# MarcoLor01/SparseMatrixVectorMultiplication

Measured on AMD Instinct MI355X. Metric: SpMV GFLOP/s (2*nnz flops / step time); achieved HBM GB/s and % of 8 TB/s alongside, higher is better.
Workload: dtype f64

## Files before the change

include/spmv_hip.h:

```cpp
#ifndef SPMV_AMD_SPMV_HIP_H
#define SPMV_AMD_SPMV_HIP_H

#include <stddef.h>

#include "csr_matrix.h"
#include "hll_matrix.h"

#ifdef __cplusplus
extern "C" {
#endif

typedef struct spmv_csr_dev spmv_csr_dev;
typedef struct spmv_hll_dev spmv_hll_dev;

enum {
    SPMV_CSR_AUTO = 0,
    SPMV_CSR_THREAD_ROW = 1,
    SPMV_CSR_WAVE_ROW = 2,
    SPMV_CSR_SUBWAVE = 3,
    SPMV_CSR_STREAM = 4
};

enum {
    SPMV_HLL_AUTO = 0,
// ... 31 lines not shown
    int tile_long_items;
    long long tile_long_entries;
    long long tile_staged_cols;
    long long tile_remainder_entries;
    int tile_mid_rows;
    int tile_mid_items;
    long long tile_mid_entries;
    int place_tries;
    float place_first_us;
    float place_best_us;
    unsigned long long val_address;
    long long tile_expanded_entries;
    long long pattern_slots;
    float pattern_with_us;
    float pattern_without_us;
} spmv_dev_info;

int spmv_hip_device_count(void);
int spmv_hip_init(int device);
int spmv_hip_shutdown(void);
int spmv_hip_sync(void);
void *spmv_hip_stream(void);
const char *spmv_hip_last_error(void);
int spmv_hip_device_name(char *buf, size_t len, int *compute_units, long long *hbm_bytes);
int spmv_hip_flush_cache(size_t bytes);
int spmv_hip_device_state(char *buf, size_t len);
int spmv_hip_stream_probe(size_t bytes, int warmup, int iters, float *ms_mean, float *ms_min);
int spmv_hip_stream_probe_at(const void *dptr, size_t bytes, int warmup, int iters, float *ms_mean, float *ms_min);
int spmv_hip_gather_probe(int value_bytes, size_t table_bytes, int waves_per_cu, double *values_per_s);
int spmv_hip_set_tuning(const char *key, int value);
// ... 10 lines not shown
                            const float *values, int row0, int row1, spmv_csr_dev **out);
int spmv_hip_csr_plan_check(int M, int N, const int *row_ptr, const int *col_idx, int value_bytes, int *stats);
int spmv_hip_csr_tile_plan_check(int M, int N, const int *row_ptr, const int *col_idx, int value_bytes,
                                 int rows_per_block, int lmax, int density, int chunk, int balance, long long *stats);
int spmv_hip_csr_tile_auto_plan(int M, int N, const int *row_ptr, const int *col_idx, int value_bytes, long long *stats);
int spmv_hip_csr_tile_digest(const spmv_csr_dev *m, unsigned long long *digest);
int spmv_hip_hll_tile_digest(const spmv_hll_dev *m, unsigned long long *digest);
int spmv_hip_csr_from_coo(int M, int N, long long nz, const int *I, const int *J, const double *val,
                          spmv_csr_dev **out);
int spmv_hip_csr_download(const spmv_csr_dev *m, int *row_ptr, int *col, void *val);
int spmv_hip_csr_upload_matrix(const CSRMatrix *csr, spmv_csr_dev **out);
void spmv_hip_csr_free(spmv_csr_dev *m);
int spmv_hip_csr_info(const spmv_csr_dev *m, spmv_dev_info *out);
int spmv_hip_csr_addresses(const spmv_csr_dev *m, unsigned long long *out);
int spmv_hip_csr_stamp_blocks(spmv_csr_dev *m, int warm, unsigned long long *stamps);
int spmv_hip_csr_relocate(spmv_csr_dev *m, int which, unsigned long long align, unsigned long long offset);
int spmv_hip_csr_relocate_vmm(spmv_csr_dev *m, int which, unsigned long long align, unsigned long long offset);

int spmv_hip_csr_set_x(spmv_csr_dev *m, const void *x_host);
int spmv_hip_csr_run(spmv_csr_dev *m, int variant);
int spmv_hip_csr_get_y(spmv_csr_dev *m, void *y_host);
void *spmv_hip_csr_x_ptr(spmv_csr_dev *m);
void *spmv_hip_csr_y_ptr(spmv_csr_dev *m);

int spmv_hip_csr_run_on(spmv_csr_dev *m, int variant, const void *d_x, void *d_y, void *stream);

int spmv_hip_csr_spmm_on(spmv_csr_dev *m, int k, const void *d_X, void *d_Y, void *stream);
int spmv_hip_csr_spmm(spmv_csr_dev *m, int k, const void *X_host, void *Y_host);
int spmv_hip_csr_spmm_time(spmv_csr_dev *m, int k, int warmup, int iters, float *ms_each);

// ... 67 lines not shown
```

sparsematrixvectormultiplication_amd/_native.py:

```python
from __future__ import annotations

import ctypes as C
import os

_HERE = os.path.dirname(os.path.abspath(__file__))
LIB_PATH = os.path.join(_HERE, "libspmv_amd.so")

c_int_p = C.POINTER(C.c_int)
c_double_p = C.POINTER(C.c_double)
c_float_p = C.POINTER(C.c_float)


class PreMatrix(C.Structure):
    _fields_ = [("M", C.c_int), ("N", C.c_int), ("nz", C.c_int), ("I", c_int_p), ("J", c_int_p),
                ("val", c_double_p), ("type", C.c_char * 4)]


class CSRMatrix(C.Structure):
    _fields_ = [("M", C.c_int), ("N", C.c_int), ("nz", C.c_int), ("row_ptr", c_int_p),
                ("col_idx", c_int_p), ("values", c_double_p), ("type", C.c_char * 4)]


class ELLPACKBlock(C.Structure):
    _fields_ = [("M", C.c_int), ("N", C.c_int), ("MAXNZ", C.c_int), ("JA", c_int_p),
# ... 11 lines not shown

class DevInfo(C.Structure):
    _fields_ = [("M_local", C.c_int), ("M_total", C.c_int), ("N", C.c_int), ("row0", C.c_int),
                ("nz", C.c_longlong), ("value_bytes", C.c_int), ("auto_variant", C.c_int),
                ("lanes_per_row", C.c_int), ("stream_blocks", C.c_int), ("long_rows", C.c_int),
                ("slots", C.c_longlong), ("hacks", C.c_int), ("algo_bytes", C.c_longlong),
                ("device_bytes", C.c_longlong), ("local_blocks", C.c_int), ("local_stage_lines", C.c_int),
                ("local_lines", C.c_longlong), ("stream_bytes", C.c_longlong), ("stream_kernel", C.c_int),
                ("tile_blocks", C.c_int), ("tile_passes", C.c_int), ("tile_split_rows", C.c_int),
                ("tile_entries", C.c_longlong), ("tile_staged_entries", C.c_longlong),
                ("tile_long_rows", C.c_int), ("tile_long_items", C.c_int), ("tile_long_entries", C.c_longlong),
                ("tile_staged_cols", C.c_longlong), ("tile_remainder_entries", C.c_longlong),
                ("tile_mid_rows", C.c_int), ("tile_mid_items", C.c_int), ("tile_mid_entries", C.c_longlong),
                ("place_tries", C.c_int), ("place_first_us", C.c_float), ("place_best_us", C.c_float),
                ("val_address", C.c_ulonglong), ("tile_expanded_entries", C.c_longlong),
                ("pattern_slots", C.c_longlong), ("pattern_with_us", C.c_float), ("pattern_without_us", C.c_float)]

    def as_dict(self):
        return {name: getattr(self, name) for name, _ in self._fields_}


_PROTOTYPES = {
    "mm_read_banner": (C.c_int, [C.c_void_p, C.c_void_p]),
    "mm_read_mtx_crd_size": (C.c_int, [C.c_void_p, c_int_p, c_int_p, c_int_p]),
    "mm_write_banner": (C.c_int, [C.c_void_p, C.c_char_p]),
    "mm_write_mtx_crd_size": (C.c_int, [C.c_void_p, C.c_int, C.c_int, C.c_int]),
    "mm_is_valid": (C.c_int, [C.c_char_p]),
    "mm_typecode_to_str": (C.c_void_p, [C.c_char_p]),
    "init_pre_matrix": (None, [C.POINTER(PreMatrix)]),
    "free_pre_matrix": (None, [C.POINTER(PreMatrix)]),
    "read_matrix_market": (C.c_int, [C.c_char_p, C.POINTER(PreMatrix)]),
# ... 59 lines not shown
    "spmv_hip_init": (C.c_int, [C.c_int]),
    "spmv_hip_shutdown": (C.c_int, []),
    "spmv_hip_sync": (C.c_int, []),
    "spmv_hip_stream": (C.c_void_p, []),
    "spmv_hip_last_error": (C.c_char_p, []),
    "spmv_hip_device_name": (C.c_int, [C.c_char_p, C.c_size_t, c_int_p, C.POINTER(C.c_longlong)]),
    "spmv_hip_flush_cache": (C.c_int, [C.c_size_t]),
    "spmv_hip_device_state": (C.c_int, [C.c_char_p, C.c_size_t]),
    "spmv_hip_stream_probe": (C.c_int, [C.c_size_t, C.c_int, C.c_int, c_float_p, c_float_p]),
    "spmv_hip_stream_probe_at": (C.c_int, [C.c_void_p, C.c_size_t, C.c_int, C.c_int, c_float_p, c_float_p]),
    "spmv_hip_gather_probe": (C.c_int, [C.c_int, C.c_size_t, C.c_int, c_double_p]),
    "spmv_hip_csr_tile_digest": (C.c_int, [C.c_void_p, C.POINTER(C.c_ulonglong)]),
    "spmv_hip_hll_tile_digest": (C.c_int, [C.c_void_p, C.POINTER(C.c_ulonglong)]),
    "spmv_hip_csr_addresses": (C.c_int, [C.c_void_p, C.POINTER(C.c_ulonglong)]),
    "spmv_hip_csr_stamp_blocks": (C.c_int, [C.c_void_p, C.c_int, C.POINTER(C.c_ulonglong)]),
    "spmv_hip_csr_relocate": (C.c_int, [C.c_void_p, C.c_int, C.c_ulonglong, C.c_ulonglong]),
    "spmv_hip_csr_relocate_vmm": (C.c_int, [C.c_void_p, C.c_int, C.c_ulonglong, C.c_ulonglong]),
    "spmv_hip_set_tuning": (C.c_int, [C.c_char_p, C.c_int]),
    "spmv_hip_malloc": (C.c_int, [C.POINTER(C.c_void_p), C.c_size_t]),
    "spmv_hip_free": (C.c_int, [C.c_void_p]),
    "spmv_hip_memcpy_h2d": (C.c_int, [C.c_void_p, C.c_void_p, C.c_size_t]),
    "spmv_hip_memcpy_d2h": (C.c_int, [C.c_void_p, C.c_void_p, C.c_size_t]),
    "spmv_hip_memset": (C.c_int, [C.c_void_p, C.c_int, C.c_size_t]),
    "spmv_hip_csr_upload": (C.c_int, [C.c_int, C.c_int, c_int_p, c_int_p, c_double_p, C.c_int,
                                      C.c_int, C.POINTER(C.c_void_p)]),
    "spmv_hip_csr_upload_f32": (C.c_int, [C.c_int, C.c_int, c_int_p, c_int_p, c_float_p, C.c_int,
                                          C.c_int, C.POINTER(C.c_void_p)]),
    "spmv_hip_csr_upload_matrix": (C.c_int, [C.POINTER(CSRMatrix), C.POINTER(C.c_void_p)]),
    "spmv_hip_csr_free": (None, [C.c_void_p]),
    "spmv_hip_csr_info": (C.c_int, [C.c_void_p, C.POINTER(DevInfo)]),
# ... 92 lines not shown
```

sparsematrixvectormultiplication_amd/csrc/hip/csr_kernels.hpp:

```cpp
#pragma once
#include <hip/hip_runtime.h>

#include <type_traits>

#include "wave_ops.hpp"

namespace spmv {

constexpr int kBlock = 256;
constexpr int kStreamCapMax = 8192;
constexpr int kStreamUnit = 2 * kBlock;
constexpr int kStreamRowsCap = 1024;
constexpr int kLongPiece = 8192;
constexpr int kBaseMask = ~3;

typedef int v2i __attribute__((ext_vector_type(2)));
typedef float v2f __attribute__((ext_vector_type(2)));
typedef double v2d __attribute__((ext_vector_type(2)));
template <typename T> struct vec2;
template <> struct vec2<float> { using type = v2f; };
template <> struct vec2<double> { using type = v2d; };

template <bool NT, typename V>
__device__ __forceinline__ V stream_load(const V *p) {
// ... 452 lines not shown
#pragma unroll
    for (int k = 0; k < ROUNDS; ++k)
        *reinterpret_cast<uint4 *>(reinterpret_cast<char *>(stage) + (k * kBlock + t) * 16) = xl[k];
    __syncthreads();
#pragma unroll
    for (int u = 0; u < kUnits; ++u) {
        const unsigned c = *reinterpret_cast<const unsigned *>(pc.slots + u * kUnit + 2 * t);
        v[u].x *= stage[c & 0xffffu];
        v[u].y *= stage[c >> 16];
    }
    __syncthreads();
#pragma unroll
    for (int u = 0; u < kUnits; ++u) *reinterpret_cast<V2 *>(&stage[u * kUnit + 2 * t]) = v[u];
}

template <typename T, bool NT, int CAP, bool STAMP = false, bool PAT = false>
__global__ __launch_bounds__(kBlock) void csr_stream_local(int num_blocks, int xcd_chunk,
                                                           const int *__restrict__ ids,
                                                           const int4 *__restrict__ desc,
                                                           const int2 *__restrict__ ldesc,
                                                           const int *__restrict__ lines,
                                                           const int *__restrict__ row_ptr,
                                                           const unsigned short *__restrict__ lcol,
                                                           const T *__restrict__ val,
                                                           const T *__restrict__ x, T *__restrict__ y,
                                                           unsigned long long *__restrict__ stamps = nullptr, int probe = 0,
                                                           const int2 *__restrict__ pdesc = nullptr,
                                                           const unsigned *__restrict__ rinfo = nullptr,
                                                           const unsigned short *__restrict__ ptab = nullptr, int stage_bytes = 0) {
        using V2 = typename vec2<T>::type;
    const bool no_slots = STAMP && (probe & 1);
    unsigned long long t_start = 0;
    if constexpr (STAMP) t_start = __builtin_amdgcn_s_memrealtime();
    constexpr int kUnit = 2 * kBlock, kUnits = CAP / kUnit;
    extern __shared__ __attribute__((aligned(16))) unsigned char local_smem[];
    T *stage = reinterpret_cast<T *>(local_smem);

    const int at = xcd_chunked(blockIdx.x, xcd_chunk);
    if (at >= num_blocks) return;
    const int b = ids ? ids[at] : at;
    const int t = threadIdx.x;
    const int4 d = desc[b];
    const int2 ld = ldesc[b];
    const int r0 = d.x, nrows = d.z;
    const int base = d.y & kBaseMask;

    const int lanes = lanes_for_rows<kBlock>(nrows);
    int seg_lo = 0, seg_hi = 0;
    if (t / lanes < nrows) {
        seg_lo = row_ptr[r0 + t / lanes];
        seg_hi = row_ptr[r0 + t / lanes + 1];
    }

    const int e_first = base + 2 * t;
    const int units = (d.w - base + kUnit - 1) / kUnit;
    const int rounds = (ld.y + kLocalLineQuantum - 1) / kLocalLineQuantum;
    const int *my_lines = lines + ld.x;
    if constexpr (PAT) {
        const int2 pd = pdesc[b];
        pat_ctx pc;
        pc.slots = reinterpret_cast<unsigned short *>(local_smem + stage_bytes);
        pc.ptab8 = reinterpret_cast<const uint4 *>(ptab + pd.x);
        pc.rinfo = rinfo;
        pc.row_ptr = row_ptr;
        pc.row_seg = nullptr;
        pc.r0 = r0;
        pc.nrows = nrows;
        pc.base = base;
        pc.first = d.y;
        pc.end = d.w;
        pc.lanes = lanes;
        pc.seg_lo = seg_lo;
        pc.seg_hi = seg_hi;
        pc.ri = t / lanes < nrows ? rinfo[r0 + t / lanes] : 0u;
        if (units == kUnits) {
            switch (rounds) {
// ... 55 lines not shown
#pragma unroll
        for (int u = 0; u < kUnits; ++u) {
            if (u < units) {
                const unsigned c = stream_load<NT>(reinterpret_cast<const unsigned *>(lcol + e_first + u * kUnit));
                p[u] = stream_load<NT>(reinterpret_cast<const V2 *>(val + e_first + u * kUnit));
                p[u].x *= stage[c & 0xffffu];
                p[u].y *= stage[c >> 16];
            }
        }
        __syncthreads();
#pragma unroll
        for (int u = 0; u < kUnits; ++u)
            if (u < units) *reinterpret_cast<V2 *>(&stage[u * kUnit + 2 * t]) = p[u];
    }
    __syncthreads();
    sum_rows_from_lds<T, kBlock>(stage, row_ptr, y, r0, nrows, base, lanes, seg_lo - base, seg_hi - base);
    if constexpr (STAMP) {
        __syncthreads();
        if (threadIdx.x == 0) {
            stamps[3 * (size_t)b] = t_start;
            stamps[3 * (size_t)b + 1] = __builtin_amdgcn_s_memrealtime();
            stamps[3 * (size_t)b + 2] = ((unsigned long long)blockIdx.x << 8) | (__builtin_amdgcn_s_getreg(20 | (3 << 11)) & 0xf);
        }
    }
}

template <typename T, bool NT>
__global__ __launch_bounds__(kBlock) void csr_long_pieces(int count, const int4 *__restrict__ pieces,
                                                          const int *__restrict__ col,
                                                          const T *__restrict__ val,
                                                          const T *__restrict__ x,
// ... 63 lines not shown
```

sparsematrixvectormultiplication_amd/csrc/hip/plan_kernels.hpp:

```cpp
#pragma once
#include <hip/hip_runtime.h>

#include <climits>

#include "csr_kernels.hpp"

namespace spmv {

constexpr int kPlanCap = 2048;
constexpr int kPlanPer = kPlanCap / kBlock;

template <int SHIFT>
__device__ __forceinline__ int sort_segment_lines(int *keys, int *scan, const int *__restrict__ idx, long long begin,
                                                  int len) {
    const int t = threadIdx.x;
#pragma unroll
    for (int j = 0; j < kPlanPer; ++j) {
        const int k = t + j * kBlock;
        keys[k] = k < len ? (idx[begin + k] >> SHIFT) : INT_MAX;
    }
    for (int size = 2; size <= kPlanCap; size <<= 1) {
        for (int stride = size >> 1; stride > 0; stride >>= 1) {
            __syncthreads();
#pragma unroll
// ... 167 lines not shown
            rinfo[r0 + i] = (unsigned)cur | ((unsigned)(shift & 0xffff) << 16);
        }
        pdesc[b] = make_int2((int)pb, filled * 8);
    }
    __syncthreads();
    for (int i = t; i < nrows; i += BLOCK) {
        if (rowflag[r0 + i] & 0x10000) continue;
        long long s;
        int len;
        pat_row_slots<HLL>(row_ptr, row_seg, base, r0 + i, s, len);
        const long long o = pb + 8 * (long long)(rinfo[r0 + i] & 0xffffu);
        for (int j = 0; j < len; ++j) ptab[o + j] = slot[s + j];
    }
}

}
```

sparsematrixvectormultiplication_amd/csrc/hip/spmv_csr.hip:

```cpp
#include "spmv_internal.hpp"

#include "plan_kernels.hpp"
#include <chrono>

#include "tile_plan.hpp"
#include "tile_plan_device.hpp"

namespace {

void csr_build_blocks(int M, const int *rp, int cap, int rows_cap, std::vector<int4> &desc,
                      std::vector<int4> &pieces, std::vector<int4> &long_rows,
                      const std::vector<unsigned char> *split = nullptr) {
    desc.clear();
    pieces.clear();
    long_rows.clear();
    auto is_long = [&](int row) { return rp[row + 1] - rp[row] > cap - 3 || (split && (*split)[row]); };
    int r = 0;
    while (r < M) {
        const int n0 = rp[r];
        const int base = n0 & kBaseMask;
        if (is_long(r)) {
            const int first_slot = (int)pieces.size();
            for (int p = n0; p < rp[r + 1]; p += kLongPiece)
                pieces.push_back(int4{r, p, std::min(p + kLongPiece, rp[r + 1]), (int)pieces.size()});
// ... 624 lines not shown
            best_us = us;
        }
        worst_us = std::max(worst_us, us);
        if (best_us < worst_us * 0.915f) break;
    }
    m->val = best;
    m->place_best_us = best_us;
    if (best != first) (void)hipFree(first);
    for (void *p : others)
        if (p != best) (void)hipFree(p);
    (void)hipEventDestroy(e0);
    (void)hipEventDestroy(e1);
    return rc;
}

int csr_build_patterns(spmv_csr_dev *m) {
    if (g_local_patterns == 0 || m->local_blocks <= 0 || !m->lcol || !m->ldesc4 || !m->row_ptr || m->M_local <= 0) return 0;
    if (g_local_patterns < 0 && (m->nz * (m->value_bytes + 2LL) <= (128LL << 20) || m->nz < 12LL * m->M_local)) return 0;
    UploadTrace trace("csr_build_patterns");
    const int B = m->local_blocks;
    int *rowflag = nullptr, *pcount = nullptr;
    long long *pbase = nullptr;
    auto drop_tmp = [&] {
        (void)hipFree(rowflag);
        (void)hipFree(pcount);
        (void)hipFree(pbase);
    };
    hipError_t e = hipMalloc((void **)&rowflag, (size_t)m->M_local * sizeof(int));
    if (e == hipSuccess) e = hipMalloc((void **)&pcount, (size_t)B * sizeof(int));
    if (e == hipSuccess) e = hipMalloc((void **)&pbase, (size_t)B * sizeof(long long));
// ... 12 lines not shown
        return fail("pattern plan: marking the rows failed: %s", hipGetErrorString(e));
    }
    std::vector<long long> h_base((size_t)B);
    long long total = 0;
    int widest = 0;
    for (int b = 0; b < B; ++b) {
        h_base[(size_t)b] = total;
        total += h_count[(size_t)b];
        widest = std::max(widest, h_count[(size_t)b]);
    }
    trace.mark("rows marked");
    if ((g_local_patterns < 0 && total * 4 > m->nz) || total > 0x7ffffff0LL) {
        drop_tmp();
        return 0;
    }
    e = hipMalloc((void **)&m->ptab, ((size_t)total + 1024) * sizeof(unsigned short));
    if (e == hipSuccess) e = hipMalloc((void **)&m->rinfo, (size_t)m->M_local * sizeof(unsigned));
    if (e == hipSuccess) e = hipMalloc((void **)&m->pdesc, (size_t)B * sizeof(int2));
    if (e == hipSuccess) e = hipMemsetAsync(m->ptab, 0, ((size_t)total + 1024) * sizeof(unsigned short), g_stream);
    if (e == hipSuccess) e = hipMemsetAsync(m->rinfo, 0, (size_t)m->M_local * sizeof(unsigned), g_stream);
    if (e == hipSuccess) e = hipMemcpyAsync(pbase, h_base.data(), (size_t)B * sizeof(long long), hipMemcpyHostToDevice, g_stream);
    if (e == hipSuccess) {
        hipLaunchKernelGGL((pat_fill<256>), dim3(B), dim3(256), 0, g_stream, B, m->ldesc4, m->row_ptr, m->lcol, rowflag, pbase, m->rinfo,
                           m->ptab, m->pdesc);
        e = hipGetLastError();
    }
    if (e == hipSuccess) e = hipStreamSynchronize(g_stream);
    drop_tmp();
    if (e != hipSuccess) {
        (void)hipFree(m->ptab);
        (void)hipFree(m->rinfo);
        (void)hipFree(m->pdesc);
        m->ptab = nullptr;
        m->rinfo = nullptr;
        m->pdesc = nullptr;
        return fail("pattern plan: building the tables failed: %s", hipGetErrorString(e));
    }
    m->pat_slots = total;
    m->pat_max = widest;
    m->device_bytes += ((size_t)total + 1024) * 2 + (size_t)m->M_local * 4 + (size_t)B * 8;
    trace.mark("tables");
    return 0;
}

int csr_tune_patterns(spmv_csr_dev *m) {
    if (g_local_patterns >= 0 || !m->ptab || !m->x || !m->y) return 0;
    hipEvent_t e0 = nullptr, e1 = nullptr;
    if (hipEventCreate(&e0) != hipSuccess || hipEventCreate(&e1) != hipSuccess) {
        if (e0) (void)hipEventDestroy(e0);
        return 0;
    }
    auto measure = [&](int patterns, float &us) {
        const int keep = g_local_patterns;
        g_local_patterns = patterns;
        int rc = 0;
        for (int i = 0; i < 2 && !rc; ++i) rc = csr_launch_any(m, SPMV_CSR_AUTO, m->x, m->y, g_stream);
// ... 8 lines not shown
        return (e == hipSuccess && !rc) ? 0 : -1;
    };
    float with_us = 0, without_us = 0;
    bool ok = true;
    for (int round = 0; round < 2 && ok; ++round) {
        float a = 0, b = 0;
        ok = measure(1, a) == 0 && measure(0, b) == 0;
        with_us = round ? std::min(with_us, a) : a;
        without_us = round ? std::min(without_us, b) : b;
    }
    (void)hipEventDestroy(e0);
    (void)hipEventDestroy(e1);
    m->pat_with_us = with_us;
    m->pat_without_us = without_us;
    if (!ok || with_us > 0.98f * without_us) {
        (void)hipFree(m->ptab);
        (void)hipFree(m->rinfo);
        (void)hipFree(m->pdesc);
        m->ptab = nullptr;
        m->rinfo = nullptr;
        m->pdesc = nullptr;
        m->device_bytes -= std::min(m->device_bytes, ((size_t)m->pat_slots + 1024) * 2 + (size_t)m->M_local * 4 + (size_t)m->local_blocks * 8);
        m->pat_slots = 0;
    }
    return 0;
}

template <typename T>
int csr_upload_impl(int M, int N, const int *row_ptr, const int *col_idx, const T *values, int row0,
                    int row1, spmv_csr_dev **out, int *adopt_col = nullptr, T *adopt_val = nullptr) {
    if (need_device()) return -1;
    if (!out) return fail("csr_upload: out is NULL");
    *out = nullptr;
    if (M < 0 || N < 0 || !row_ptr) return fail("csr_upload: bad arguments");
    if (row0 < 0 || row1 < row0 || row1 > M) return fail("csr_upload: bad row range [%d, %d) of %d", row0, row1, M);
    const int Ml = row1 - row0;
    const int e0 = row_ptr[row0], e1 = row_ptr[row1];
    const long long nz = (long long)e1 - e0;
// ... 617 lines not shown
    for (auto &r : m->relocs) {
        *r.field = nullptr;
        release_relocated(r);
    }
    (void)hipFree(m->row_ptr);
    (void)hipFree(m->col);
    (void)hipFree(m->val);
    (void)hipFree(m->desc);
    (void)hipFree(m->ldesc4);
    (void)hipFree(m->ldesc);
    (void)hipFree(m->lines);
    (void)hipFree(m->lcol);
    (void)hipFree(m->ptab);
    (void)hipFree(m->rinfo);
    (void)hipFree(m->pdesc);
    for (spmv_csr_dev::long_tiles *tier : {&m->mt}) {
        (void)hipFree(tier->block_row);
        (void)hipFree(tier->block_pass);
        (void)hipFree(tier->block_of_row);
        (void)hipFree(tier->item_first);
        (void)hipFree(tier->row_map);
        (void)hipFree(tier->pass);
        (void)hipFree(tier->work);
        (void)hipFree(tier->tcol);
        (void)hipFree(tier->tkey);
        (void)hipFree(tier->tval);
        (void)hipFree(tier->slab);
    }
    (void)hipFree(m->lt.block_row);
    (void)hipFree(m->lt.block_pass);
// ... 229 lines not shown
    out->tile_long_rows = m->lt.rows;
    out->tile_long_entries = m->lt.entries;
    out->tile_staged_cols = m->tile_staged_cols + m->lt.staged_cols + m->mt.staged_cols;
    out->tile_long_items = m->lt.items;
    out->tile_mid_rows = m->mt.rows;
    out->tile_mid_entries = m->mt.entries;
    out->tile_mid_items = m->mt.items;
    out->place_tries = m->place_tries;
    out->place_first_us = m->place_first_us;
    out->place_best_us = m->place_best_us;
    out->val_address = (unsigned long long)(uintptr_t)m->val;
    out->tile_expanded_entries = m->xe && m->expansion ? (long long)m->expansion->entries : 0;
    out->pattern_slots = m->ptab ? m->pat_slots : 0;
    out->pattern_with_us = m->pat_with_us;
    out->pattern_without_us = m->pat_without_us;
    out->stream_kernel = m->local_blocks > 0 ? 1 : m->tile_blocks > 0 ? 3
                         : ((m->stream_cap == 4096 || m->stream_cap == 2048) && m->M_local > 0 &&
                            m->nz < (long long)m->M_local * (m->stream_cap / kBlock)) ? 2 : 0;
    if (m->local_blocks > 0)
        out->stream_bytes = m->nz * vb + (m->ptab ? 2 * m->pat_slots + 4LL * m->M_local + 8LL * m->local_blocks : 2 * m->nz) +
                            4 * m->local_lines + 24LL * m->local_blocks + 4LL * (m->M_local + 1) + vb * m->M_local + vb * m->N;
    else if (m->tile_blocks > 0) {
        out->stream_bytes = m->tile_padded * (vb + 6) - (m->tile_packed ? 2 : 0) * m->tile_staged + 16LL * m->tile_passes +
                            4LL * m->tile_blocks +
                            std::max<long long>(0, m->nz - m->tile_entries - m->tile_rem_entries - m->lt.entries - m->mt.entries) * (vb + 4) +
                            m->tile_rem_entries * (vb + 4) + 16LL * m->tile_num_pieces + vb * m->M_local + vb * m->N;
        if (m->xe && m->expansion)
            out->stream_bytes += (long long)m->expansion->entries * (2 * vb) + 24LL * m->expansion->chunks +
                                 4LL * (long long)(m->expansion->runs + m->expansion->groups);
        for (const spmv_csr_dev::long_tiles *tier : {&m->lt, &m->mt})
            out->stream_bytes += tier->padded * (vb + 6) - (tier->packed ? 2 : 0) * tier->staged + 16LL * tier->passes +
                                 2 * vb * (long long)tier->items * tier->rows_per_block;
    }
    return 0;
}

// ... 143 lines not shown
                                           m->tile_num_pieces, m->tile_pieces, m->col, (const T *)m->val, x, (T *)m->partial);
                        hipLaunchKernelGGL((csr_long_finish<T>), dim3(m->tile_num_long), dim3(64), 0, s, m->tile_num_long,
                                           m->tile_long_rows, (const T *)m->partial, y);
                    }
                    HIP_TRY(hipGetLastError());
                    return 0;
                }
                if (local) {
                    const int lcount = part < 0 ? m->local_blocks : part == 0 ? m->num_interior : m->num_boundary;
                    const int *lids = part < 0 ? nullptr : part == 0 ? m->interior_ids : m->boundary_ids;
                    const int lchunk = g_stream_xcd < 0 ? (lcount + 7) / 8 : (g_stream_xcd ? g_stream_xcd : 16);
                    const int lgrid = lchunk > 0 ? (lcount + 8 * lchunk - 1) / (8 * lchunk) * (8 * lchunk) : lcount;
                    if (lcount > 0) {
                    const size_t lds = std::max((size_t)m->local_cap * sizeof(T), (size_t)m->local_stage_lines * kLineBytes);
                    const bool patterns = m->ptab && m->rinfo && m->pdesc && g_local_patterns != 0;
                    const size_t pat_lds = lds + ((size_t)m->local_cap + 8) * sizeof(unsigned short);
#define SPMV_LOCAL(NT, CAP)                                                                                   \
    do {                                                                                                      \
        if (patterns)                                                                                         \
            hipLaunchKernelGGL((csr_stream_local<T, NT, CAP, false, true>), dim3(lgrid), dim3(kBlock), pat_lds, s, lcount, lchunk, \
                               lids, m->ldesc4, m->ldesc, m->lines, m->row_ptr, m->lcol, (const T *)m->val, x, y, \
                               (unsigned long long *)nullptr, 0, m->pdesc, m->rinfo, m->ptab, (int)lds);       \
        else                                                                                                  \
            hipLaunchKernelGGL((csr_stream_local<T, NT, CAP>), dim3(lgrid), dim3(kBlock), lds, s, lcount, lchunk, lids, \
                               m->ldesc4, m->ldesc, m->lines, m->row_ptr, m->lcol, (const T *)m->val, x, y);   \
    } while (0)
                    const bool lnt = g_local_nt < 0 ? m->nz * (long long)(sizeof(T) + 2) > (128LL << 20) : g_local_nt != 0;
                    if (m->local_cap == 1024) { if (lnt) SPMV_LOCAL(true, 1024); else SPMV_LOCAL(false, 1024); }
                    else if (m->local_cap == 3072) { if (lnt) SPMV_LOCAL(true, 3072); else SPMV_LOCAL(false, 3072); }
                    else { if (lnt) SPMV_LOCAL(true, 2048); else SPMV_LOCAL(false, 2048); }
                    }
#undef SPMV_LOCAL
#ifdef SPMV_EXPERIMENTAL
                } else if (g_stream_kind == 4 && m->ring_ok) {
                    const int wgs = std::max(1, std::min(g_num_cus * g_pipe_wgs_per_cu, m->num_blocks));
                    if (g_pipe_wgs_per_cu >= 2) {
                        if (g_stream_nt) hipLaunchKernelGGL((csr_stream_ring<T, true, 3, 2>), dim3(wgs), dim3(kRingBlock), 0, s, m->num_blocks, SPMV_ARGS);
// ... 279 lines not shown
```

sparsematrixvectormultiplication_amd/csrc/hip/spmv_internal.hpp:

```cpp
#pragma once
#include <hip/hip_runtime.h>
#include <rccl/rccl.h>

#include <algorithm>
#include <cstdarg>
#include <cstdio>
#include <cstdlib>
#include <cstring>
#include <ctime>
#include <new>
#include <string>
#include <vector>

#include "csr_kernels.hpp"
#ifdef SPMV_EXPERIMENTAL
#include "csr_kernels_experimental.hpp"
#endif
#include "hll_kernels.hpp"
#include "tile_kernels.hpp"
#include "spmv_hip.h"

using namespace spmv;

extern int g_device;
// ... 139 lines not shown
    int num_long = 0;
    int4 *pieces = nullptr;
    void *partial = nullptr;
    int num_partial = 0;
    void *spmm_partial = nullptr;
    size_t spmm_partial_bytes = 0;
    int stream_cap = 2048;
    bool ring_ok = false;
    int4 *ldesc4 = nullptr;
    int2 *ldesc = nullptr;
    int *lines = nullptr;
    unsigned short *lcol = nullptr;
    unsigned short *ptab = nullptr;
    unsigned *rinfo = nullptr;
    int2 *pdesc = nullptr;
    long long pat_slots = 0;
    int pat_max = 0;
    float pat_with_us = 0, pat_without_us = 0;
    int local_blocks = 0;
    int local_stage_lines = 0;
    int local_cap = 2048;
    long long local_lines = 0;
    int *interior_ids = nullptr, *boundary_ids = nullptr;
    int num_interior = 0, num_boundary = 0;
    bool have_split = false;
    spmv_csr_dev *own_part = nullptr, *halo_part = nullptr;
    long long own_entries = 0, halo_entries = 0;
    bool tiles_only = false;
    int tile_blocks = 0;
    int tile_rows = 0;
    int tile_chunk = 0;
    bool tile_packed = false;
// ... 215 lines not shown
```

Baseline: 1103.

## Pack per-block pattern metadata into contiguous segments staged once in LDS

For each local stream block, the row info, row offsets and pattern table groups are packed into one contiguous uint4 segment at plan time. The kernel loads this segment with a single coalesced read, expands column slots from it in LDS, and sums rows from the segment offsets instead of reading row_ptr and rinfo separately. In the full-block path the x gathers are issued asynchronously through global_load_lds and overlap the slot expansion. Segments are capped by an LDS budget chosen to keep the same workgroups per CU, so extra LDS and plan memory are traded for fewer scattered metadata reads.

```diff
diff --git a/include/spmv_hip.h b/include/spmv_hip.h
--- a/include/spmv_hip.h
+++ b/include/spmv_hip.h
@@ -69,6 +69,9 @@
     long long pattern_slots;
     float pattern_with_us;
     float pattern_without_us;
+    int pattern_segment_max;
+    int pattern_segment_cap;
+    long long pattern_table_rows;
 } spmv_dev_info;
 
 int spmv_hip_device_count(void);
@@ -109,6 +112,7 @@
 int spmv_hip_csr_info(const spmv_csr_dev *m, spmv_dev_info *out);
 int spmv_hip_csr_addresses(const spmv_csr_dev *m, unsigned long long *out);
 int spmv_hip_csr_stamp_blocks(spmv_csr_dev *m, int warm, unsigned long long *stamps);
+int spmv_hip_csr_pattern_segment_cap(int value_bytes, int local_cap, int stage_lines);
 int spmv_hip_csr_relocate(spmv_csr_dev *m, int which, unsigned long long align, unsigned long long offset);
 int spmv_hip_csr_relocate_vmm(spmv_csr_dev *m, int which, unsigned long long align, unsigned long long offset);
 
diff --git a/sparsematrixvectormultiplication_amd/_native.py b/sparsematrixvectormultiplication_amd/_native.py
--- a/sparsematrixvectormultiplication_amd/_native.py
+++ b/sparsematrixvectormultiplication_amd/_native.py
@@ -49,7 +49,8 @@
                 ("tile_mid_rows", C.c_int), ("tile_mid_items", C.c_int), ("tile_mid_entries", C.c_longlong),
                 ("place_tries", C.c_int), ("place_first_us", C.c_float), ("place_best_us", C.c_float),
                 ("val_address", C.c_ulonglong), ("tile_expanded_entries", C.c_longlong),
-                ("pattern_slots", C.c_longlong), ("pattern_with_us", C.c_float), ("pattern_without_us", C.c_float)]
+                ("pattern_slots", C.c_longlong), ("pattern_with_us", C.c_float), ("pattern_without_us", C.c_float),
+                ("pattern_segment_max", C.c_int), ("pattern_segment_cap", C.c_int), ("pattern_table_rows", C.c_longlong)]
 
     def as_dict(self):
         return {name: getattr(self, name) for name, _ in self._fields_}
@@ -139,6 +140,7 @@
     "spmv_hip_hll_tile_digest": (C.c_int, [C.c_void_p, C.POINTER(C.c_ulonglong)]),
     "spmv_hip_csr_addresses": (C.c_int, [C.c_void_p, C.POINTER(C.c_ulonglong)]),
     "spmv_hip_csr_stamp_blocks": (C.c_int, [C.c_void_p, C.c_int, C.POINTER(C.c_ulonglong)]),
+    "spmv_hip_csr_pattern_segment_cap": (C.c_int, [C.c_int, C.c_int, C.c_int]),
     "spmv_hip_csr_relocate": (C.c_int, [C.c_void_p, C.c_int, C.c_ulonglong, C.c_ulonglong]),
     "spmv_hip_csr_relocate_vmm": (C.c_int, [C.c_void_p, C.c_int, C.c_ulonglong, C.c_ulonglong]),
     "spmv_hip_set_tuning": (C.c_int, [C.c_char_p, C.c_int]),
diff --git a/sparsematrixvectormultiplication_amd/csrc/hip/csr_kernels.hpp b/sparsematrixvectormultiplication_amd/csrc/hip/csr_kernels.hpp
--- a/sparsematrixvectormultiplication_amd/csrc/hip/csr_kernels.hpp
+++ b/sparsematrixvectormultiplication_amd/csrc/hip/csr_kernels.hpp
@@ -490,6 +490,127 @@
     for (int u = 0; u < kUnits; ++u) *reinterpret_cast<V2 *>(&stage[u * kUnit + 2 * t]) = v[u];
 }
 
+typedef __attribute__((address_space(3))) void seg_lds_void;
+typedef const __attribute__((address_space(1))) void seg_glb_void;
+__host__ __device__ __forceinline__ int seg_groups_at(int nrows) { return (4 * nrows + 2 * (nrows + 1) + 15) >> 4; }
+
+template <int BLOCK, int CAP>
+__device__ __forceinline__ void seg_zero_outside(unsigned short *slots, int first_rel, int end_rel) {
+    const int t = threadIdx.x;
+    constexpr int kUnit = 2 * BLOCK;
+#pragma unroll
+    for (int u = 0; u < CAP / kUnit; ++u) {
+        const int e = u * kUnit + 2 * t;
+        if (e < first_rel || e >= end_rel) slots[e] = 0;
+        if (e + 1 < first_rel || e + 1 >= end_rel) slots[e + 1] = 0;
+    }
+}
+__device__ __forceinline__ void seg_write_group(unsigned short *q, int left, const uint4 p, int shift) {
+    const unsigned shift2 = ((unsigned)shift & 0xffffu) * 0x10001u;
+    unsigned a = pat_shifted(p.x, shift2), b = pat_shifted(p.y, shift2), c = pat_shifted(p.z, shift2), d = pat_shifted(p.w, shift2);
+    if (left >= 8) {
+        const uint4 w = make_uint4(a, b, c, d);
+        __builtin_memcpy(q, &w, 16);
+        return;
+    }
+    if (left & 4) {
+        const uint2 w = make_uint2(a, b);
+        __builtin_memcpy(q, &w, 8);
+        q += 4;
+        a = c;
+        b = d;
+    }
+    if (left & 2) {
+        __builtin_memcpy(q, &a, 4);
+        q += 2;
+        a = b;
+    }
+    if (left & 1) *q = (unsigned short)a;
+}
+template <int BLOCK>
+__device__ __forceinline__ void seg_expand_slots(unsigned short *slots, const uint4 *seg, int nrows, int lanes) {
+    const int t = threadIdx.x;
+    const int my_row = t / lanes, my_lane = t % lanes, rows_per_pass = BLOCK / lanes;
+    const unsigned *info = reinterpret_cast<const unsigned *>(seg);
+    const unsigned short *lo = reinterpret_cast<const unsigned short *>(info + nrows);
+    const uint4 *grp = seg + seg_groups_at(nrows);
+    for (int row = my_row; row < nrows; row += rows_per_pass) {
+        const int a = lo[row], len = lo[row + 1] - a;
+        const unsigned ri = info[row];
+        const int off = (int)(ri & 0xffffu), shift = (int)(short)(ri >> 16);
+        for (int g = my_lane; g * 8 < len; g += lanes) seg_write_group(slots + a + g * 8, len - g * 8, grp[off + g], shift);
+    }
+}
+
+__device__ __forceinline__ void lds_barrier() { asm volatile("s_waitcnt lgkmcnt(0)\n\ts_barrier" ::: "memory"); }
+
+template <typename T, int BLOCK>
+__device__ __forceinline__ void seg_sum_rows(const T *prod, const uint4 *seg, T *__restrict__ y, int r0, int nrows,
+                                             int lanes) {
+    const int t = threadIdx.x;
+    const int rows_per_pass = BLOCK / lanes;
+    const int my_row = t / lanes, my_lane = t % lanes;
+    const unsigned short *lo = reinterpret_cast<const unsigned short *>(reinterpret_cast<const unsigned *>(seg) + nrows);
+    for (int first = 0; first < nrows; first += rows_per_pass) {
+        const int row = first + my_row;
+        int a = 0, z = 0;
+        if (row < nrows) {
+            a = lo[row];
+            z = lo[row + 1];
+        }
+        T acc = lds_strided_sum(prod, a, z, my_lane, lanes);
+        acc = group_sum_rt(acc, lanes);
+        if (my_lane == 0 && row < nrows) y[r0 + row] = acc;
+    }
+}
+
+template <typename T, bool NT, int CAP, int ROUNDS>
+__device__ __forceinline__ void local_stage_full_seg(T *stage, const int *__restrict__ my_lines, int last_line,
+                                                     const T *__restrict__ val, const T *__restrict__ x, int e_first,
+                                                     unsigned short *slots, uint4 *seg_lds, const uint4 *__restrict__ seg,
+                                                     int seg_len, int nrows, int lanes, int first_rel, int end_rel) {
+    using V2 = typename vec2<T>::type;
+    constexpr int kUnit = 2 * kBlock, kUnits = CAP / kUnit;
+    const int t = threadIdx.x;
+    int line[ROUNDS];
+#pragma unroll
+    for (int k = 0; k < ROUNDS; ++k) {
+        const int at = k * kLocalLineQuantum + (t >> 3);
+        line[k] = stream_load<NT>(my_lines + (k == ROUNDS - 1 ? min(at, last_line) : at));
+    }
+    uint4 sg = make_uint4(0, 0, 0, 0);
+    if (t < seg_len) sg = seg[t];
+    V2 v[kUnits];
+#pragma unroll
+    for (int u = 0; u < kUnits; ++u) v[u] = stream_load<NT>(reinterpret_cast<const V2 *>(val + e_first + u * kUnit));
+    __builtin_amdgcn_sched_barrier(0);
+    const int wave = __builtin_amdgcn_readfirstlane(t >> 6);
+    unsigned off[ROUNDS];
+#pragma unroll
+    for (int k = 0; k < ROUNDS; ++k) off[k] = (unsigned)line[k] * (unsigned)kLineBytes + (unsigned)(t & 7) * 16u;
+    __builtin_amdgcn_sched_barrier(0);
+#pragma unroll
+    for (int k = 0; k < ROUNDS; ++k)
+        __builtin_amdgcn_global_load_lds((seg_glb_void *)(reinterpret_cast<const char *>(x) + off[k]),
+                                         (seg_lds_void *)(reinterpret_cast<char *>(stage) + (k * kBlock + wave * 64) * 16), 16, 0, 0);
+    __builtin_amdgcn_sched_barrier(0);
+    seg_zero_outside<kBlock, CAP>(slots, first_rel, end_rel);
+    if (t < seg_len) seg_lds[t] = sg;
+    lds_barrier();
+    seg_expand_slots<kBlock>(slots, seg_lds, nrows, lanes);
+    asm volatile("s_waitcnt vmcnt(0)" ::: "memory");
+    __syncthreads();
+#pragma unroll
+    for (int u = 0; u < kUnits; ++u) {
+        const unsigned c = *reinterpret_cast<const unsigned *>(slots + u * kUnit + 2 * t);
+        v[u].x *= stage[c & 0xffffu];
+        v[u].y *= stage[c >> 16];
+    }
+    __syncthreads();
+#pragma unroll
+    for (int u = 0; u < kUnits; ++u) *reinterpret_cast<V2 *>(&stage[u * kUnit + 2 * t]) = v[u];
+}
+
 template <typename T, bool NT, int CAP, bool STAMP = false, bool PAT = false>
 __global__ __launch_bounds__(kBlock) void csr_stream_local(int num_blocks, int xcd_chunk,
                                                            const int *__restrict__ ids,
@@ -503,7 +624,9 @@
                                                            unsigned long long *__restrict__ stamps = nullptr, int probe = 0,
                                                            const int2 *__restrict__ pdesc = nullptr,
                                                            const unsigned *__restrict__ rinfo = nullptr,
-                                                           const unsigned short *__restrict__ ptab = nullptr, int stage_bytes = 0) {
+                                                           const unsigned short *__restrict__ ptab = nullptr, int stage_bytes = 0,
+                                                           const int2 *__restrict__ sdesc = nullptr,
+                                                           const uint4 *__restrict__ pseg = nullptr) {
         using V2 = typename vec2<T>::type;
     const bool no_slots = STAMP && (probe & 1);
     unsigned long long t_start = 0;
@@ -520,10 +643,13 @@
     const int2 ld = ldesc[b];
     const int r0 = d.x, nrows = d.z;
     const int base = d.y & kBaseMask;
+    int2 sd = make_int2(0, 0);
+    if (PAT && sdesc) sd = sdesc[b];
+    const bool seg = PAT && sd.y > 0;
 
     const int lanes = lanes_for_rows<kBlock>(nrows);
     int seg_lo = 0, seg_hi = 0;
-    if (t / lanes < nrows) {
+    if (!seg && t / lanes < nrows) {
         seg_lo = row_ptr[r0 + t / lanes];
         seg_hi = row_ptr[r0 + t / lanes + 1];
     }
@@ -532,10 +658,58 @@
     const int units = (d.w - base + kUnit - 1) / kUnit;
     const int rounds = (ld.y + kLocalLineQuantum - 1) / kLocalLineQuantum;
     const int *my_lines = lines + ld.x;
-    if constexpr (PAT) {
+    unsigned short *slots = reinterpret_cast<unsigned short *>(local_smem + stage_bytes);
+    uint4 *seg_lds = reinterpret_cast<uint4 *>(local_smem + stage_bytes + (CAP + 8) * sizeof(unsigned short));
+    if (seg) {
+        const uint4 *sp = pseg + sd.x;
+        const int first_rel = d.y - base, end_rel = d.w - base;
+        if (units == kUnits) {
+#define SPMV_SEG(R) local_stage_full_seg<T, NT, CAP, R>(stage, my_lines, ld.y - 1, val, x, e_first, slots, seg_lds, sp, sd.y, \
+                                                        nrows, lanes, first_rel, end_rel)
+            switch (rounds) {
+                case 1: SPMV_SEG(1); break;
+                case 2: SPMV_SEG(2); break;
+                case 3: SPMV_SEG(3); break;
+                case 4: SPMV_SEG(4); break;
+                case 5: SPMV_SEG(5); break;
+                case 6: SPMV_SEG(6); break;
+                case 7: SPMV_SEG(7); break;
+                default: SPMV_SEG(8); break;
+            }
+#undef SPMV_SEG
+        } else {
+            uint4 sg = make_uint4(0, 0, 0, 0);
+            if (t < sd.y) sg = sp[t];
+            for (int k = 0; k < rounds; ++k) {
+                const int line = my_lines[min(k * kLocalLineQuantum + (t >> 3), ld.y - 1)];
+                const unsigned off = (unsigned)line * (unsigned)kLineBytes + (unsigned)(t & 7) * 16u;
+                *reinterpret_cast<uint4 *>(reinterpret_cast<char *>(stage) + (k * kBlock + t) * 16) =
+                    *reinterpret_cast<const uint4 *>(reinterpret_cast<const char *>(x) + off);
+            }
+            seg_zero_outside<kBlock, CAP>(slots, first_rel, end_rel);
+            if (t < sd.y) seg_lds[t] = sg;
+            __syncthreads();
+            seg_expand_slots<kBlock>(slots, seg_lds, nrows, lanes);
+            __syncthreads();
+            V2 p[kUnits];
+#pragma unroll
+            for (int u = 0; u < kUnits; ++u) {
+                if (u < units) {
+                    const unsigned c = *reinterpret_cast<const unsigned *>(slots + u * kUnit + 2 * t);
+                    p[u] = stream_load<NT>(reinterpret_cast<const V2 *>(val + e_first + u * kUnit));
+                    p[u].x *= stage[c & 0xffffu];
+                    p[u].y *= stage[c >> 16];
+                }
+            }
+            __syncthreads();
+#pragma unroll
+            for (int u = 0; u < kUnits; ++u)
+                if (u < units) *reinterpret_cast<V2 *>(&stage[u * kUnit + 2 * t]) = p[u];
+        }
+    } else if constexpr (PAT) {
         const int2 pd = pdesc[b];
         pat_ctx pc;
-        pc.slots = reinterpret_cast<unsigned short *>(local_smem + stage_bytes);
+        pc.slots = slots;
         pc.ptab8 = reinterpret_cast<const uint4 *>(ptab + pd.x);
         pc.rinfo = rinfo;
         pc.row_ptr = row_ptr;
@@ -621,7 +795,8 @@
             if (u < units) *reinterpret_cast<V2 *>(&stage[u * kUnit + 2 * t]) = p[u];
     }
     __syncthreads();
-    sum_rows_from_lds<T, kBlock>(stage, row_ptr, y, r0, nrows, base, lanes, seg_lo - base, seg_hi - base);
+    if (seg) seg_sum_rows<T, kBlock>(stage, seg_lds, y, r0, nrows, lanes);
+    else sum_rows_from_lds<T, kBlock>(stage, row_ptr, y, r0, nrows, base, lanes, seg_lo - base, seg_hi - base);
     if constexpr (STAMP) {
         __syncthreads();
         if (threadIdx.x == 0) {
diff --git a/sparsematrixvectormultiplication_amd/csrc/hip/plan_kernels.hpp b/sparsematrixvectormultiplication_amd/csrc/hip/plan_kernels.hpp
--- a/sparsematrixvectormultiplication_amd/csrc/hip/plan_kernels.hpp
+++ b/sparsematrixvectormultiplication_amd/csrc/hip/plan_kernels.hpp
@@ -205,4 +205,25 @@
     }
 }
 
-}
+template <int BLOCK>
+__global__ __launch_bounds__(BLOCK) void pat_segment(int blocks, const int4 *__restrict__ desc, const int *__restrict__ row_ptr,
+                                                     const unsigned *__restrict__ rinfo, const unsigned short *__restrict__ ptab,
+                                                     const int2 *__restrict__ tdesc, const int2 *__restrict__ sdesc,
+                                                     uint4 *__restrict__ seg) {
+    const int b = blockIdx.x, t = threadIdx.x;
+    if (b >= blocks) return;
+    const int2 sd = sdesc[b];
+    if (sd.y <= 0) return;
+    const int4 d = desc[b];
+    const int r0 = d.x, nrows = d.z, base = d.y & kBaseMask;
+    unsigned *info = reinterpret_cast<unsigned *>(seg + sd.x);
+    unsigned short *lo = reinterpret_cast<unsigned short *>(info + nrows);
+    uint4 *grp = seg + sd.x + seg_groups_at(nrows);
+    for (int i = t; i < nrows; i += BLOCK) info[i] = rinfo[r0 + i];
+    for (int i = t; i <= nrows; i += BLOCK) lo[i] = (unsigned short)(row_ptr[r0 + i] - base);
+    const int2 td = tdesc[b];
+    const uint4 *tab = reinterpret_cast<const uint4 *>(ptab + td.x);
+    for (int g = t; g < td.y / 8; g += BLOCK) grp[g] = tab[g];
+}
+
+}
diff --git a/sparsematrixvectormultiplication_amd/csrc/hip/spmv_csr.hip b/sparsematrixvectormultiplication_amd/csrc/hip/spmv_csr.hip
--- a/sparsematrixvectormultiplication_amd/csrc/hip/spmv_csr.hip
+++ b/sparsematrixvectormultiplication_amd/csrc/hip/spmv_csr.hip
@@ -662,6 +662,27 @@
     return rc;
 }
 
+constexpr size_t kLdsPerCu = 160 * 1024, kLdsGranule = 512;
+constexpr int kLocalWgsPerCu = 7;
+static int pattern_segment_cap(int value_bytes, int local_cap, int stage_lines) {
+    const size_t stage = std::max((size_t)local_cap * (size_t)value_bytes, (size_t)stage_lines * kLineBytes);
+    const size_t fixed = stage + ((size_t)local_cap + 8) * sizeof(unsigned short);
+    auto per_cu = [](size_t bytes) { return kLdsPerCu / ((bytes + kLdsGranule - 1) / kLdsGranule * kLdsGranule); };
+    const size_t want = std::min((size_t)kLocalWgsPerCu, per_cu(fixed));
+    int cap = 0;
+    while (cap < kBlock && per_cu(fixed + (size_t)(cap + 1) * sizeof(uint4)) >= want) ++cap;
+    return cap;
+}
+int csr_pattern_segment_cap(const spmv_csr_dev *m) {
+    return pattern_segment_cap(m->value_bytes, m->local_cap, m->local_stage_lines);
+}
+extern "C" int spmv_hip_csr_pattern_segment_cap(int value_bytes, int local_cap, int stage_lines) {
+    if ((value_bytes != 4 && value_bytes != 8) || local_cap <= 0 || local_cap > kStreamCapMax || stage_lines < 0 ||
+        stage_lines > kLocalLinesMax)
+        return fail("csr_pattern_segment_cap: bad arguments (%d, %d, %d)", value_bytes, local_cap, stage_lines);
+    return 16 * pattern_segment_cap(value_bytes, local_cap, stage_lines);
+}
+
 int csr_build_patterns(spmv_csr_dev *m) {
     if (g_local_patterns == 0 || m->local_blocks <= 0 || !m->lcol || !m->ldesc4 || !m->row_ptr || m->M_local <= 0) return 0;
     if (g_local_patterns < 0 && (m->nz * (m->value_bytes + 2LL) <= (128LL << 20) || m->nz < 12LL * m->M_local)) return 0;
@@ -704,6 +725,18 @@
         drop_tmp();
         return 0;
     }
+    auto drop_plan = [&] {
+        (void)hipFree(m->ptab);
+        (void)hipFree(m->rinfo);
+        (void)hipFree(m->pdesc);
+        (void)hipFree(m->pseg);
+        (void)hipFree(m->sdesc);
+        m->ptab = nullptr;
+        m->rinfo = nullptr;
+        m->pdesc = nullptr;
+        m->pseg = nullptr;
+        m->sdesc = nullptr;
+    };
     e = hipMalloc((void **)&m->ptab, ((size_t)total + 1024) * sizeof(unsigned short));
     if (e == hipSuccess) e = hipMalloc((void **)&m->rinfo, (size_t)m->M_local * sizeof(unsigned));
     if (e == hipSuccess) e = hipMalloc((void **)&m->pdesc, (size_t)B * sizeof(int2));
@@ -715,21 +748,59 @@
                            m->ptab, m->pdesc);
         e = hipGetLastError();
     }
+    std::vector<int4> h_desc((size_t)B);
+    if (e == hipSuccess) e = hipMemcpyAsync(h_desc.data(), m->ldesc4, (size_t)B * sizeof(int4), hipMemcpyDeviceToHost, g_stream);
     if (e == hipSuccess) e = hipStreamSynchronize(g_stream);
     drop_tmp();
     if (e != hipSuccess) {
-        (void)hipFree(m->ptab);
-        (void)hipFree(m->rinfo);
-        (void)hipFree(m->pdesc);
-        m->ptab = nullptr;
-        m->rinfo = nullptr;
-        m->pdesc = nullptr;
+        drop_plan();
         return fail("pattern plan: building the tables failed: %s", hipGetErrorString(e));
+    }
+    trace.mark("tables");
+    const int cap16 = csr_pattern_segment_cap(m);
+    std::vector<int2> h_sdesc((size_t)B, make_int2(0, 0));
+    long long seg_total = 0, table_rows = 0;
+    int seg_max = 0;
+    for (int b = 0; b < B; ++b) {
+        const int4 d = h_desc[(size_t)b];
+        const int len = seg_groups_at(d.z) + h_count[(size_t)b] / 8;
+        if (len <= cap16) {
+            h_sdesc[(size_t)b] = make_int2((int)seg_total, len);
+            seg_total += len;
+            seg_max = std::max(seg_max, len);
+        } else {
+            table_rows += d.z;
+        }
+    }
+    if (seg_max > 0 && seg_total <= 0x7fffffffLL) {
+        e = hipMalloc((void **)&m->pseg, (size_t)seg_total * sizeof(uint4));
+        if (e == hipSuccess) e = hipMalloc((void **)&m->sdesc, (size_t)B * sizeof(int2));
+        if (e == hipSuccess) e = hipMemsetAsync(m->pseg, 0, (size_t)seg_total * sizeof(uint4), g_stream);
+        if (e == hipSuccess) e = hipMemcpyAsync(m->sdesc, h_sdesc.data(), (size_t)B * sizeof(int2), hipMemcpyHostToDevice, g_stream);
+        if (e == hipSuccess) {
+            hipLaunchKernelGGL((pat_segment<256>), dim3(B), dim3(256), 0, g_stream, B, m->ldesc4, m->row_ptr, m->rinfo, m->ptab,
+                               m->pdesc, m->sdesc, m->pseg);
+            e = hipGetLastError();
+        }
+        if (e == hipSuccess) e = hipStreamSynchronize(g_stream);
+        if (e != hipSuccess) {
+            drop_plan();
+            return fail("pattern plan: building the segments failed: %s", hipGetErrorString(e));
+        }
+    } else {
+        seg_total = 0;
+        seg_max = 0;
+        table_rows = m->M_local;
     }
     m->pat_slots = total;
     m->pat_max = widest;
+    m->pat_seg_total = seg_total;
+    m->pat_seg_max = seg_max;
+    m->pat_seg_cap = cap16;
+    m->pat_table_rows = table_rows;
     m->device_bytes += ((size_t)total + 1024) * 2 + (size_t)m->M_local * 4 + (size_t)B * 8;
-    trace.mark("tables");
+    if (m->pseg) m->device_bytes += (size_t)seg_total * sizeof(uint4) + (size_t)B * sizeof(int2);
+    trace.mark("segments");
     return 0;
 }
 
@@ -768,14 +839,22 @@
     m->pat_with_us = with_us;
     m->pat_without_us = without_us;
     if (!ok || with_us > 0.98f * without_us) {
+        m->device_bytes -= std::min(m->device_bytes, ((size_t)m->pat_slots + 1024) * 2 + (size_t)m->M_local * 4 + (size_t)m->local_blocks * 8 +
+                                                          (m->pseg ? (size_t)m->pat_seg_total * sizeof(uint4) + (size_t)m->local_blocks * sizeof(int2) : 0));
         (void)hipFree(m->ptab);
         (void)hipFree(m->rinfo);
         (void)hipFree(m->pdesc);
+        (void)hipFree(m->pseg);
+        (void)hipFree(m->sdesc);
         m->ptab = nullptr;
         m->rinfo = nullptr;
         m->pdesc = nullptr;
-        m->device_bytes -= std::min(m->device_bytes, ((size_t)m->pat_slots + 1024) * 2 + (size_t)m->M_local * 4 + (size_t)m->local_blocks * 8);
+        m->pseg = nullptr;
+        m->sdesc = nullptr;
         m->pat_slots = 0;
+        m->pat_seg_total = 0;
+        m->pat_seg_max = 0;
+        m->pat_table_rows = 0;
     }
     return 0;
 }
@@ -1423,6 +1502,8 @@
     (void)hipFree(m->ptab);
     (void)hipFree(m->rinfo);
     (void)hipFree(m->pdesc);
+    (void)hipFree(m->pseg);
+    (void)hipFree(m->sdesc);
     for (spmv_csr_dev::long_tiles *tier : {&m->mt}) {
         (void)hipFree(tier->block_row);
         (void)hipFree(tier->block_pass);
@@ -1682,12 +1763,17 @@
     out->pattern_slots = m->ptab ? m->pat_slots : 0;
     out->pattern_with_us = m->pat_with_us;
     out->pattern_without_us = m->pat_without_us;
+    out->pattern_segment_max = m->ptab ? 16 * m->pat_seg_max : 0;
+    out->pattern_segment_cap = 16 * m->pat_seg_cap;
+    out->pattern_table_rows = m->ptab ? m->pat_table_rows : 0;
     out->stream_kernel = m->local_blocks > 0 ? 1 : m->tile_blocks > 0 ? 3
                          : ((m->stream_cap == 4096 || m->stream_cap == 2048) && m->M_local > 0 &&
                             m->nz < (long long)m->M_local * (m->stream_cap / kBlock)) ? 2 : 0;
     if (m->local_blocks > 0)
-        out->stream_bytes = m->nz * vb + (m->ptab ? 2 * m->pat_slots + 4LL * m->M_local + 8LL * m->local_blocks : 2 * m->nz) +
-                            4 * m->local_lines + 24LL * m->local_blocks + 4LL * (m->M_local + 1) + vb * m->M_local + vb * m->N;
+        out->stream_bytes = m->nz * vb + (m->ptab ? 16 * m->pat_seg_total + 8LL * m->local_blocks +
+                                                        (2 * m->pat_slots + 8LL * m->M_local) * m->pat_table_rows / std::max(1, m->M_local)
+                                                  : 2 * m->nz + 4LL * (m->M_local + 1)) +
+                            4 * m->local_lines + 24LL * m->local_blocks + vb * m->M_local + vb * m->N;
     else if (m->tile_blocks > 0) {
         out->stream_bytes = m->tile_padded * (vb + 6) - (m->tile_packed ? 2 : 0) * m->tile_staged + 16LL * m->tile_passes +
                             4LL * m->tile_blocks +
@@ -1861,13 +1947,13 @@
                     if (lcount > 0) {
                     const size_t lds = std::max((size_t)m->local_cap * sizeof(T), (size_t)m->local_stage_lines * kLineBytes);
                     const bool patterns = m->ptab && m->rinfo && m->pdesc && g_local_patterns != 0;
-                    const size_t pat_lds = lds + ((size_t)m->local_cap + 8) * sizeof(unsigned short);
+                    const size_t pat_lds = lds + ((size_t)m->local_cap + 8) * sizeof(unsigned short) + (size_t)m->pat_seg_max * sizeof(uint4);
 #define SPMV_LOCAL(NT, CAP)                                                                                   \
     do {                                                                                                      \
         if (patterns)                                                                                         \
             hipLaunchKernelGGL((csr_stream_local<T, NT, CAP, false, true>), dim3(lgrid), dim3(kBlock), pat_lds, s, lcount, lchunk, \
                                lids, m->ldesc4, m->ldesc, m->lines, m->row_ptr, m->lcol, (const T *)m->val, x, y, \
-                               (unsigned long long *)nullptr, 0, m->pdesc, m->rinfo, m->ptab, (int)lds);       \
+                               (unsigned long long *)nullptr, 0, m->pdesc, m->rinfo, m->ptab, (int)lds, m->sdesc, (const uint4 *)m->pseg); \
         else                                                                                                  \
             hipLaunchKernelGGL((csr_stream_local<T, NT, CAP>), dim3(lgrid), dim3(kBlock), lds, s, lcount, lchunk, lids, \
                                m->ldesc4, m->ldesc, m->lines, m->row_ptr, m->lcol, (const T *)m->val, x, y);   \
diff --git a/sparsematrixvectormultiplication_amd/csrc/hip/spmv_internal.hpp b/sparsematrixvectormultiplication_amd/csrc/hip/spmv_internal.hpp
--- a/sparsematrixvectormultiplication_amd/csrc/hip/spmv_internal.hpp
+++ b/sparsematrixvectormultiplication_amd/csrc/hip/spmv_internal.hpp
@@ -177,8 +177,14 @@
     unsigned short *ptab = nullptr;
     unsigned *rinfo = nullptr;
     int2 *pdesc = nullptr;
+    uint4 *pseg = nullptr;
+    int2 *sdesc = nullptr;
     long long pat_slots = 0;
     int pat_max = 0;
+    long long pat_seg_total = 0;
+    int pat_seg_max = 0;
+    int pat_seg_cap = 0;
+    long long pat_table_rows = 0;
     float pat_with_us = 0, pat_without_us = 0;
     int local_blocks = 0;
     int local_stage_lines = 0;
```

After: 1216, median of 6. +10.2%, better.
